# genlm/genlm-backend

Hardware: AMD Instinct MI355X
Metric: particles/sec + logprob-kernel HBM GB/s (% of 8 TB/s), 1024 particles gpt2 (higher is better)
Workload: dtype f32

## Files before the change

genlm-backend_amd/csrc/glb_kv.hip:

```cpp
#include <hip/hip_runtime.h>

#include <climits>

#include "../../include/glb.h"
#include "glb_common.hpp"

namespace {

__device__ inline uint64_t ctx_hash_step(uint64_t h, uint32_t v) {
  h ^= v;
  h *= 0x100000001b3ull;
  return h ^ (h >> 29);
}

__global__ __launch_bounds__(64) void match_rows_kernel(const int32_t *tok, const int64_t *st, const int32_t *len,
                                                        const int32_t *rep, const int32_t *n_groups, const int32_t *row_tok,
                                                        const int32_t *row_len, const uint64_t *row_hash, int32_t R,
                                                        int32_t cap, int32_t *out_old, uint64_t *out_hash) {
  const int u = blockIdx.x, lane = threadIdx.x;
  if (u >= *n_groups) return;
  const int i = rep[u];
  const int32_t L = len[i];
  const int32_t *t = tok + st[i];
  uint64_t h = 0xcbf29ce484222325ull, h_par = h;
// ... 499 lines not shown
  const int p0_new = a.pos[r], nn = a.n_new[r];
  const int64_t sr = a.row_of ? (int64_t)a.row_of[r] : (int64_t)r;
  char *out = a.out + ((((int64_t)r * a.T + t) * a.H + h) * DH + i * EPV) * ES;
  const bool bad = p0_new < 0 || nn < 1 || nn > a.T || (int64_t)p0_new + nn > a.cap || sr < 0 || sr >= a.n_slab_rows;
  if (bad || t >= nn) {
    if (j == 0) {
      float z[EPV];
#pragma unroll
      for (int k = 0; k < EPV; ++k) z[k] = bad ? __builtin_nanf("") : 0.0f;
      *reinterpret_cast<u32x4 *>(out) = pack16v<DT>(z);
    }
    return;
  }
  const int p_new = p0_new + t;
  float qf[EPV];
  unpack16<DT>(*reinterpret_cast<const u32x4 *>(a.q + ((int64_t)r * a.q_sr + (int64_t)h * a.q_sh + (int64_t)t * a.q_sp + i * EPV) * ES), qf);
  const char *kb = a.k_new + ((int64_t)r * a.k_sr + (int64_t)hk * a.k_sh + i * EPV) * ES;
  const char *vb = a.v_new + ((int64_t)r * a.v_sr + (int64_t)hk * a.v_sh + i * EPV) * ES;
  const int64_t slab_row = (sr * a.Hkv + hk) * a.cap;
  if (h == hk * G && j == 0) {
    *reinterpret_cast<u32x4 *>(a.k_slab + ((slab_row + p_new) * DH + i * EPV) * ES) = *reinterpret_cast<const u32x4 *>(kb + (int64_t)t * a.k_sp * ES);
    *reinterpret_cast<u32x4 *>(a.v_slab + ((slab_row + p_new) * DH + i * EPV) * ES) = *reinterpret_cast<const u32x4 *>(vb + (int64_t)t * a.v_sp * ES);
  }
  float m = -__builtin_huge_valf(), l = 0.0f, acc[EPV];
#pragma unroll
  for (int k = 0; k < EPV; ++k) acc[k] = 0.0f;
  for (int p0 = 0; p0 <= p_new; p0 += PP) {
    const int p = p0 + j;
    float kf[EPV], vf[EPV];
    if (p < p0_new) {
      unpack16<DT>(*reinterpret_cast<const u32x4 *>(a.k_slab + ((slab_row + p) * DH + i * EPV) * ES), kf);
      unpack16<DT>(*reinterpret_cast<const u32x4 *>(a.v_slab + ((slab_row + p) * DH + i * EPV) * ES), vf);
    } else {
      const int tn = p <= p_new ? p - p0_new : t;
      unpack16<DT>(*reinterpret_cast<const u32x4 *>(kb + (int64_t)tn * a.k_sp * ES), kf);
      unpack16<DT>(*reinterpret_cast<const u32x4 *>(vb + (int64_t)tn * a.v_sp * ES), vf);
    }
    float s = 0.0f;
#pragma unroll
    for (int k = 0; k < EPV; ++k) s = __builtin_fmaf(qf[k], kf[k], s);
#pragma unroll
    for (int o = 1; o < LP; o <<= 1) s += __shfl_xor(s, o, 64);
    if (p <= p_new) {
      s *= a.scale;
      const float m2 = fmaxf(m, s), c = __expf(m - m2), w = __expf(s - m2);
      l = l * c + w;
#pragma unroll
      for (int k = 0; k < EPV; ++k) acc[k] = __builtin_fmaf(acc[k], c, w * vf[k]);
      m = m2;
    }
  }
#pragma unroll
  for (int o = LP; o < 64; o <<= 1) {
    const float mo = __shfl_xor(m, o, 64), lo = __shfl_xor(l, o, 64);
    const float m2 = fmaxf(m, mo);
    const float c = m == m2 ? 1.0f : __expf(m - m2), co = mo == m2 ? 1.0f : __expf(mo - m2);
    l = l * c + lo * co;
#pragma unroll
    for (int k = 0; k < EPV; ++k) acc[k] = acc[k] * c + __shfl_xor(acc[k], o, 64) * co;
    m = m2;
  }
  if (j == 0) {
    const float inv = 1.0f / l;
#pragma unroll
    for (int k = 0; k < EPV; ++k) acc[k] *= inv;
    *reinterpret_cast<u32x4 *>(out) = pack16v<DT>(acc);
  }
}

template <int DT>
hipError_t launch_attention_chunk(const ChunkAttnArgs &a, int head_dim, hipStream_t s) {
  const dim3 grid((unsigned)((int64_t)a.n * a.H * a.T)), block(64);
  if (head_dim == 64) hipLaunchKernelGGL((slab_attention_chunk_kernel<DT, 64>), grid, block, 0, s, a);
  else if (head_dim == 128) hipLaunchKernelGGL((slab_attention_chunk_kernel<DT, 128>), grid, block, 0, s, a);
  else if (head_dim == 32) hipLaunchKernelGGL((slab_attention_chunk_kernel<DT, 32>), grid, block, 0, s, a);
  else if (head_dim == 16) hipLaunchKernelGGL((slab_attention_chunk_kernel<DT, 16>), grid, block, 0, s, a);
  else return hipErrorInvalidValue;
  return hipGetLastError();
}

struct ShortArgs {
  const char *q, *k, *v;
  const uint8_t *mask;
  char *out;
  int64_t q_sr, q_sh, q_sp, k_sr, k_sh, k_sp, v_sr, v_sh, v_sp, m_sr, m_sq;
  int32_t U, H, Hkv, Lq, Lk;
  float scale;
};

template <int DT, int DH>
__global__ __launch_bounds__(64) void short_attention_kernel(const ShortArgs a) {
  constexpr int ES = DT == GLB_F32 ? 4 : 2, EPV = 16 / ES, LP = DH / EPV, PP = 64 / LP;
  static_assert(LP >= 1 && LP <= 64 && PP * LP == 64, "head_dim / vector width must divide the wave");
  const int lane = threadIdx.x, j = lane / LP, i = lane - j * LP;
  const int t = blockIdx.x % a.Lq, uh = blockIdx.x / a.Lq, h = uh % a.H, u = uh / a.H;
  const int hk = h / (a.H / a.Hkv);
  float qf[EPV];
  unpack16<DT>(*reinterpret_cast<const u32x4 *>(a.q + ((int64_t)u * a.q_sr + (int64_t)h * a.q_sh + (int64_t)t * a.q_sp + i * EPV) * ES), qf);
  const uint8_t *mrow = a.mask ? a.mask + (int64_t)u * a.m_sr + (int64_t)t * a.m_sq : nullptr;
  const int last = mrow ? a.Lk - 1 : (t + a.Lk - a.Lq < a.Lk - 1 ? t + a.Lk - a.Lq : a.Lk - 1);
  const char *kb = a.k + ((int64_t)u * a.k_sr + (int64_t)hk * a.k_sh + i * EPV) * ES;
  const char *vb = a.v + ((int64_t)u * a.v_sr + (int64_t)hk * a.v_sh + i * EPV) * ES;
  float m = -__builtin_huge_valf(), l = 0.0f, acc[EPV];
#pragma unroll
  for (int k = 0; k < EPV; ++k) acc[k] = 0.0f;
  for (int p0 = 0; p0 <= last; p0 += PP) {
    const int p = p0 + j;
    const bool in = p <= last;
    const bool see = in && (mrow ? mrow[p] != 0 : true);
    float kf[EPV], vf[EPV];
    const int pc = in ? p : last;
    unpack16<DT>(*reinterpret_cast<const u32x4 *>(kb + (int64_t)pc * a.k_sp * ES), kf);
    unpack16<DT>(*reinterpret_cast<const u32x4 *>(vb + (int64_t)pc * a.v_sp * ES), vf);
    float s = 0.0f;
#pragma unroll
    for (int k = 0; k < EPV; ++k) s = __builtin_fmaf(qf[k], kf[k], s);
#pragma unroll
    for (int o = 1; o < LP; o <<= 1) s += __shfl_xor(s, o, 64);
    if (see) {
      s *= a.scale;
      const float m2 = fmaxf(m, s), c = __expf(m - m2), w = __expf(s - m2);
      l = l * c + w;
#pragma unroll
      for (int k = 0; k < EPV; ++k) acc[k] = __builtin_fmaf(acc[k], c, w * vf[k]);
      m = m2;
    }
  }
#pragma unroll
  for (int o = LP; o < 64; o <<= 1) {
    const float mo = __shfl_xor(m, o, 64), lo = __shfl_xor(l, o, 64);
    const float m2 = fmaxf(m, mo);
    const float c = m == m2 ? 1.0f : __expf(m - m2), co = mo == m2 ? 1.0f : __expf(mo - m2);
    l = l * c + lo * co;
#pragma unroll
    for (int k = 0; k < EPV; ++k) acc[k] = acc[k] * c + __shfl_xor(acc[k], o, 64) * co;
    m = m2;
  }
  if (j == 0) {
    const float inv = l > 0.0f ? 1.0f / l : 0.0f;
#pragma unroll
    for (int k = 0; k < EPV; ++k) acc[k] *= inv;
    *reinterpret_cast<u32x4 *>(a.out + ((((int64_t)u * a.Lq + t) * a.H + h) * DH + i * EPV) * ES) = pack16v<DT>(acc);
  }
}

template <int LP>
__device__ __forceinline__ float slot_sum(float v) {
  if constexpr (LP >= 2) v += __uint_as_float((uint32_t)__builtin_amdgcn_update_dpp(0, (int)__float_as_uint(v), 0xB1, 0xf, 0xf, false));
  if constexpr (LP >= 4) v += __uint_as_float((uint32_t)__builtin_amdgcn_update_dpp(0, (int)__float_as_uint(v), 0x4E, 0xf, 0xf, false));
  if constexpr (LP >= 8) v += __uint_as_float((uint32_t)__builtin_amdgcn_update_dpp(0, (int)__float_as_uint(v), 0x141, 0xf, 0xf, false));
  if constexpr (LP >= 16) v += __uint_as_float((uint32_t)__builtin_amdgcn_update_dpp(0, (int)__float_as_uint(v), 0x140, 0xf, 0xf, false));
  if constexpr (LP >= 32) v += __shfl_xor(v, 16, 64);
  if constexpr (LP >= 64) v += __shfl_xor(v, 32, 64);
  return v;
}

template <int DT, int DH, int KMAX>
__global__ __launch_bounds__(64) void short_attention_rows_kernel(const ShortArgs a) {
  constexpr int ES = DT == GLB_F32 ? 4 : 2, EPV = 16 / ES, LP = DH / EPV, PP = 64 / LP;
  static_assert(LP >= 1 && LP <= 64 && PP * LP == 64, "head_dim / vector width must divide the wave");
  constexpr bool KREG = KMAX * EPV <= 128;
  extern __shared__ float kv_lds[];
  const int lane = threadIdx.x, j = lane / LP, i = lane - j * LP;
  const int G = a.H / a.Hkv;
  const int hk = blockIdx.x % a.Hkv, u = blockIdx.x / a.Hkv;
  float *Ks = kv_lds, *Vs = KREG ? kv_lds : kv_lds + a.Lk * DH;
  const char *kb = a.k + ((int64_t)u * a.k_sr + (int64_t)hk * a.k_sh) * ES;
  const char *vb = a.v + ((int64_t)u * a.v_sr + (int64_t)hk * a.v_sh) * ES;
  const int nq = G * a.Lq;
  auto q_addr = [&](int qi) {
    const int qc = qi < nq ? qi : nq - 1;
    const int g = qc / a.Lq, t = qc - g * a.Lq;
    return a.q + ((int64_t)u * a.q_sr + (int64_t)(hk * G + g) * a.q_sh + (int64_t)t * a.q_sp + i * EPV) * ES;
  };
  u32x4 q_raw = *reinterpret_cast<const u32x4 *>(q_addr(j));
  float kr[KREG ? KMAX : 1][EPV];
  if constexpr (KREG) {
    u32x4 raw[KMAX];
#pragma unroll
    for (int p = 0; p < KMAX; ++p)
      raw[p] = *reinterpret_cast<const u32x4 *>(kb + ((int64_t)(p < a.Lk ? p : 0) * a.k_sp + i * EPV) * ES);
#pragma unroll
    for (int p = 0; p < KMAX; ++p) unpack16<DT>(raw[p], kr[p]);
  }
  for (int x = lane; x < a.Lk * LP; x += 64) {
    const int p = x / LP, c = x - p * LP;
    float vf[EPV];
    unpack16<DT>(*reinterpret_cast<const u32x4 *>(vb + ((int64_t)p * a.v_sp + c * EPV) * ES), vf);
#pragma unroll
    for (int k = 0; k < EPV; ++k) Vs[p * DH + c * EPV + k] = vf[k];
    if constexpr (!KREG) {
      float kf[EPV];
      unpack16<DT>(*reinterpret_cast<const u32x4 *>(kb + ((int64_t)p * a.k_sp + c * EPV) * ES), kf);
#pragma unroll
      for (int k = 0; k < EPV; ++k) Ks[p * DH + c * EPV + k] = kf[k];
    }
  }
  const uint32_t all_keys = a.Lk >= 32 ? 0xffffffffu : ((1u << a.Lk) - 1u);
  uint32_t *vis_t = reinterpret_cast<uint32_t *>(kv_lds + (KREG ? 1 : 2) * a.Lk * DH);
  for (int t = lane; t < a.Lq; t += 64) {
    uint32_t vis = 0;
    if (a.mask) {
      const uint8_t *mrow = a.mask + (int64_t)u * a.m_sr + (int64_t)t * a.m_sq;
      uint8_t mb[KMAX];
#pragma unroll
      for (int p = 0; p < KMAX; ++p) mb[p] = p < a.Lk ? mrow[p] : (uint8_t)0;
#pragma unroll
      for (int p = 0; p < KMAX; ++p) vis |= (mb[p] != 0 ? 1u : 0u) << p;
    } else {
      const int last = t + a.Lk - a.Lq;
      vis = last >= 31 ? 0xffffffffu : ((2u << last) - 1u);
    }
    vis_t[t] = vis & all_keys;
  }
  __syncthreads();
  for (int q0 = 0; q0 < nq; q0 += PP) {
    const int qi = q0 + j;
    const bool live = qi < nq;
    const int qc = live ? qi : nq - 1;
    const int g = qc / a.Lq, t = qc - g * a.Lq, h = hk * G + g;
    float qf[EPV];
    unpack16<DT>(q_raw, qf);
    if (q0 + PP < nq) q_raw = *reinterpret_cast<const u32x4 *>(q_addr(qi + PP));
    const uint32_t vis = vis_t[t];
    float sc[KMAX];
    float m = -__builtin_huge_valf();
#pragma unroll
    for (int p = 0; p < KMAX; ++p) {
      sc[p] = -__builtin_huge_valf();
      if (p < a.Lk) {
        float s = 0.0f;
        if constexpr (KREG) {
#pragma unroll
          for (int k = 0; k < EPV; ++k) s = __builtin_fmaf(qf[k], kr[p][k], s);
        } else {
          const float *kp = Ks + p * DH + i * EPV;
#pragma unroll
          for (int k = 0; k < EPV; ++k) s = __builtin_fmaf(qf[k], kp[k], s);
        }
        s = slot_sum<LP>(s) * a.scale;
        sc[p] = ((vis >> p) & 1u) ? s : -__builtin_huge_valf();
        m = fmaxf(m, sc[p]);
      }
    }
    float l = 0.0f, acc[EPV];
#pragma unroll
    for (int k = 0; k < EPV; ++k) acc[k] = 0.0f;
#pragma unroll
    for (int p = 0; p < KMAX; ++p) {
      if (p < a.Lk) {
        const float w = ((vis >> p) & 1u) ? __expf(sc[p] - m) : 0.0f;
        const float *vp = Vs + p * DH + i * EPV;
        l += w;
#pragma unroll
        for (int k = 0; k < EPV; ++k) acc[k] = __builtin_fmaf(w, vp[k], acc[k]);
      }
    }
    if (live) {
      const float inv = l > 0.0f ? 1.0f / l : 0.0f;
#pragma unroll
      for (int k = 0; k < EPV; ++k) acc[k] *= inv;
      *reinterpret_cast<u32x4 *>(a.out + ((((int64_t)u * a.Lq + t) * a.H + h) * DH + i * EPV) * ES) = pack16v<DT>(acc);
    }
  }
}

template <int DT, int DH>
hipError_t launch_short_rows(const ShortArgs &a, hipStream_t s) {
  const dim3 grid((unsigned)((int64_t)a.U * a.Hkv)), block(64);
  const size_t lds = (size_t)2 * a.Lk * DH * sizeof(float) + (size_t)a.Lq * sizeof(uint32_t);
  if (a.Lk <= 16) hipLaunchKernelGGL((short_attention_rows_kernel<DT, DH, 16>), grid, block, lds, s, a);
  else hipLaunchKernelGGL((short_attention_rows_kernel<DT, DH, 32>), grid, block, lds, s, a);
  return hipGetLastError();
}

template <int DT>
hipError_t launch_short_attention(const ShortArgs &a, int head_dim, hipStream_t s) {
  if (a.Lk <= 32 && a.Lq <= 2048 && (int64_t)a.U * a.Hkv <= 0x7fffffffll) {
    if (head_dim == 64) return launch_short_rows<DT, 64>(a, s);
    if (head_dim == 128) return launch_short_rows<DT, 128>(a, s);
    if (head_dim == 32) return launch_short_rows<DT, 32>(a, s);
    if (head_dim == 16) return launch_short_rows<DT, 16>(a, s);
    return hipErrorInvalidValue;
  }
  const dim3 grid((unsigned)((int64_t)a.U * a.H * a.Lq)), block(64);
  if (head_dim == 64) hipLaunchKernelGGL((short_attention_kernel<DT, 64>), grid, block, 0, s, a);
  else if (head_dim == 128) hipLaunchKernelGGL((short_attention_kernel<DT, 128>), grid, block, 0, s, a);
  else if (head_dim == 32) hipLaunchKernelGGL((short_attention_kernel<DT, 32>), grid, block, 0, s, a);
  else if (head_dim == 16) hipLaunchKernelGGL((short_attention_kernel<DT, 16>), grid, block, 0, s, a);
  else return hipErrorInvalidValue;
  return hipGetLastError();
}

struct PackedArgs {
  const char *q, *k, *v;
  char *out;
  const int32_t *plan;
  uint32_t *err;
  int64_t q_sr, q_sh, k_sr, k_sh, v_sr, v_sh;
  int32_t S, M, H, Hkv, max_keys;
  float scale;
};

template <int DT, int DH, int KMAX>
__global__ __launch_bounds__(64) void short_attention_packed_kernel(const PackedArgs a) {
  constexpr int ES = DT == GLB_F32 ? 4 : 2, EPV = 16 / ES, LP = DH / EPV, PP = 64 / LP;
  static_assert(LP >= 1 && LP <= 64 && PP * LP == 64, "head_dim / vector width must divide the wave");
  constexpr bool KREG = KMAX * EPV <= 128;
  extern __shared__ float kv_lds[];
  const int lane = threadIdx.x, j = lane / LP, i = lane - j * LP;
  const int G = a.H / a.Hkv;
  const int hk = blockIdx.x % a.Hkv, s = blockIdx.x / a.Hkv;
  if (s >= a.S) return;
  const int32_t *seg = a.plan + (int64_t)s * 4;
  const int64_t pre_start = seg[0], pre_len = seg[1], tail_start = seg[2], tail_len = seg[3];
  const int64_t n_keys = pre_len + tail_len;
  if (pre_len < 0 || tail_len < 1 || n_keys > a.max_keys || n_keys > KMAX || pre_start < 0 || pre_start + pre_len > a.M ||
      tail_start < 0 || tail_start + tail_len > a.M) {
    if (lane == 0 && hk == 0) atomicAdd(a.err, 1u);
    return;
  }
  const int Lk = (int)n_keys, Lq = (int)tail_len, pre = (int)pre_len;
  auto key_row = [&](int p) -> int64_t { return p < pre ? pre_start + p : tail_start + (p - pre); };
  float *Ks = kv_lds, *Vs = KREG ? kv_lds : kv_lds + Lk * DH;
  const char *kb = a.k + (int64_t)hk * a.k_sh * ES;
  const char *vb = a.v + (int64_t)hk * a.v_sh * ES;
  const int nq = G * Lq;
  auto q_addr = [&](int qi) {
    const int qc = qi < nq ? qi : nq - 1;
    const int g = qc / Lq, t = qc - g * Lq;
    return a.q + ((tail_start + t) * a.q_sr + (int64_t)(hk * G + g) * a.q_sh + i * EPV) * ES;
  };
  u32x4 q_raw = *reinterpret_cast<const u32x4 *>(q_addr(j));
  float kr[KREG ? KMAX : 1][EPV];
  if constexpr (KREG) {
    u32x4 raw[KMAX];
#pragma unroll
    for (int p = 0; p < KMAX; ++p)
      raw[p] = *reinterpret_cast<const u32x4 *>(kb + (key_row(p < Lk ? p : 0) * a.k_sr + i * EPV) * ES);
#pragma unroll
    for (int p = 0; p < KMAX; ++p) unpack16<DT>(raw[p], kr[p]);
  }
  for (int x = lane; x < Lk * LP; x += 64) {
    const int p = x / LP, c = x - p * LP;
    const int64_t row = key_row(p);
    float vf[EPV];
    unpack16<DT>(*reinterpret_cast<const u32x4 *>(vb + (row * a.v_sr + c * EPV) * ES), vf);
#pragma unroll
    for (int k = 0; k < EPV; ++k) Vs[p * DH + c * EPV + k] = vf[k];
    if constexpr (!KREG) {
      float kf[EPV];
      unpack16<DT>(*reinterpret_cast<const u32x4 *>(kb + (row * a.k_sr + c * EPV) * ES), kf);
#pragma unroll
      for (int k = 0; k < EPV; ++k) Ks[p * DH + c * EPV + k] = kf[k];
    }
  }
  const uint32_t all_keys = Lk >= 32 ? 0xffffffffu : ((1u << Lk) - 1u);
  uint32_t *vis_t = reinterpret_cast<uint32_t *>(kv_lds + (KREG ? 1 : 2) * Lk * DH);
  for (int t = lane; t < Lq; t += 64) {
    const int last = t + pre;
    const uint32_t vis = last >= 31 ? 0xffffffffu : ((2u << last) - 1u);
    vis_t[t] = vis & all_keys;
  }
  __syncthreads();
  for (int q0 = 0; q0 < nq; q0 += PP) {
    const int qi = q0 + j;
    const bool live = qi < nq;
    const int qc = live ? qi : nq - 1;
    const int g = qc / Lq, t = qc - g * Lq, h = hk * G + g;
    float qf[EPV];
    unpack16<DT>(q_raw, qf);
    if (q0 + PP < nq) q_raw = *reinterpret_cast<const u32x4 *>(q_addr(qi + PP));
    const uint32_t vis = vis_t[t];
    float sc[KMAX];
    float m = -__builtin_huge_valf();
#pragma unroll
    for (int p = 0; p < KMAX; ++p) {
      sc[p] = -__builtin_huge_valf();
      if (p < Lk) {
        float sv = 0.0f;
        if constexpr (KREG) {
#pragma unroll
          for (int k = 0; k < EPV; ++k) sv = __builtin_fmaf(qf[k], kr[p][k], sv);
        } else {
          const float *kp = Ks + p * DH + i * EPV;
#pragma unroll
          for (int k = 0; k < EPV; ++k) sv = __builtin_fmaf(qf[k], kp[k], sv);
        }
        sv = slot_sum<LP>(sv) * a.scale;
        sc[p] = ((vis >> p) & 1u) ? sv : -__builtin_huge_valf();
        m = fmaxf(m, sc[p]);
      }
    }
    float l = 0.0f, acc[EPV];
#pragma unroll
    for (int k = 0; k < EPV; ++k) acc[k] = 0.0f;
#pragma unroll
    for (int p = 0; p < KMAX; ++p) {
      if (p < Lk) {
        const float w = ((vis >> p) & 1u) ? __expf(sc[p] - m) : 0.0f;
        const float *vp = Vs + p * DH + i * EPV;
        l += w;
#pragma unroll
        for (int k = 0; k < EPV; ++k) acc[k] = __builtin_fmaf(w, vp[k], acc[k]);
      }
    }
    if (live) {
      const float inv = l > 0.0f ? 1.0f / l : 0.0f;
#pragma unroll
      for (int k = 0; k < EPV; ++k) acc[k] *= inv;
      *reinterpret_cast<u32x4 *>(a.out + (((tail_start + t) * a.H + h) * DH + i * EPV) * ES) = pack16v<DT>(acc);
    }
  }
}

template <int DT, int DH>
hipError_t launch_short_packed_dh(const PackedArgs &a, hipStream_t s) {
  const dim3 grid((unsigned)((int64_t)a.S * a.Hkv)), block(64);
  const size_t lds = (size_t)2 * a.max_keys * DH * sizeof(float) + (size_t)a.max_keys * sizeof(uint32_t);
  if (a.max_keys <= 16) hipLaunchKernelGGL((short_attention_packed_kernel<DT, DH, 16>), grid, block, lds, s, a);
  else hipLaunchKernelGGL((short_attention_packed_kernel<DT, DH, 32>), grid, block, lds, s, a);
  return hipGetLastError();
}

template <int DT>
hipError_t launch_short_packed(const PackedArgs &a, int head_dim, hipStream_t s) {
  if (head_dim == 64) return launch_short_packed_dh<DT, 64>(a, s);
  if (head_dim == 128) return launch_short_packed_dh<DT, 128>(a, s);
  if (head_dim == 32) return launch_short_packed_dh<DT, 32>(a, s);
  if (head_dim == 16) return launch_short_packed_dh<DT, 16>(a, s);
  return hipErrorInvalidValue;
}


template <typename VT>
__global__ void kv_append_kernel(VT *slab, const VT *rows, const int32_t *pos, const int32_t *row_of, int64_t n_rows,
                                 int64_t heads, int64_t cap, int64_t row_vecs, int64_t rows_stride_row,
                                 int64_t rows_stride_head) {
  const int64_t gid = (int64_t)blockIdx.x * blockDim.x + threadIdx.x;
  if (gid >= n_rows * heads * row_vecs) return;
  const int64_t x = gid % row_vecs, h = (gid / row_vecs) % heads, i = gid / (row_vecs * heads);
  const int64_t p = pos[i], r = row_of ? (int64_t)row_of[i] : i;
  if (p < 0 || p >= cap || r < 0) return;
  slab[((r * heads + h) * cap + p) * row_vecs + x] = rows[i * rows_stride_row + h * rows_stride_head + x];
}

template <typename VT>
__global__ void kv_gather_rows_kernel(const VT *const *src, VT *const *dst, int64_t n_rows, int64_t heads,
                                      int64_t row_vecs, int64_t src_cap, int64_t dst_cap, const int32_t *src_row_of,
                                      const int32_t *len_of) {
  const int t = blockIdx.y;
  const int64_t gid = (int64_t)blockIdx.x * blockDim.x + threadIdx.x;
  const int64_t per_row = heads * dst_cap * row_vecs;
  if (gid >= n_rows * per_row) return;
  const int64_t i = gid / per_row, r = gid % per_row;
  const int64_t x = r % row_vecs, p = (r / row_vecs) % dst_cap, h = r / (row_vecs * dst_cap);
  const int64_t sr = src_row_of[i];
  if (sr < 0 || p >= len_of[i] || p >= src_cap) return;
  dst[t][((i * heads + h) * dst_cap + p) * row_vecs + x] = src[t][((sr * heads + h) * src_cap + p) * row_vecs + x];
}

__global__ void gather_rows_i32_kernel(const int32_t *src, int64_t src_ld, const int32_t *row_of, int64_t n,
                                       int64_t width, int32_t *dst, int64_t dst_ld) {
  const int64_t gid = (int64_t)blockIdx.x * blockDim.x + threadIdx.x;
  if (gid >= n * width) return;
  const int64_t i = gid / width, j = gid % width;
  dst[i * dst_ld + j] = src[(int64_t)row_of[i] * src_ld + j];
}


}

extern "C" {

int glb_kv_append(void *slab, const void *new_rows, const int32_t *pos, const int32_t *row_of, int64_t n_rows,
                  int64_t heads, int64_t cap, int64_t head_dim, int64_t new_stride_row, int64_t new_stride_head,
                  int32_t elem_bytes, void *stream) {
  if (!slab || !new_rows || !pos) return glb::api_fail(GLB_EINVAL, "null pointer");
  if (n_rows <= 0 || heads <= 0 || cap <= 0 || head_dim <= 0) return glb::api_fail(GLB_EINVAL, "bad sizes");
  if (elem_bytes != 2 && elem_bytes != 4) return glb::api_fail(GLB_EINVAL, "elem_bytes must be 2 or 4");
  const int64_t rowb = head_dim * elem_bytes;
  hipStream_t s = (hipStream_t)stream;
  const bool wide = rowb % 16 == 0 && ((uintptr_t)slab) % 16 == 0 && ((uintptr_t)new_rows) % 16 == 0 &&
                    (new_stride_row * elem_bytes) % 16 == 0 && (new_stride_head * elem_bytes) % 16 == 0;
  if (wide) {
    const int64_t rv = rowb / 16, total = n_rows * heads * rv;
    hipLaunchKernelGGL(kv_append_kernel<uint4>, dim3(blocks_for(total, 256)), dim3(256), 0, s, (uint4 *)slab,
                       (const uint4 *)new_rows, pos, row_of, n_rows, heads, cap, rv, new_stride_row * elem_bytes / 16,
                       new_stride_head * elem_bytes / 16);
  } else if (elem_bytes == 4) {
    const int64_t total = n_rows * heads * head_dim;
    hipLaunchKernelGGL(kv_append_kernel<uint32_t>, dim3(blocks_for(total, 256)), dim3(256), 0, s, (uint32_t *)slab,
                       (const uint32_t *)new_rows, pos, row_of, n_rows, heads, cap, head_dim, new_stride_row, new_stride_head);
  } else {
    const int64_t total = n_rows * heads * head_dim;
    hipLaunchKernelGGL(kv_append_kernel<uint16_t>, dim3(blocks_for(total, 256)), dim3(256), 0, s, (uint16_t *)slab,
                       (const uint16_t *)new_rows, pos, row_of, n_rows, heads, cap, head_dim, new_stride_row, new_stride_head);
  }
  const hipError_t e = hipGetLastError();
  if (e != hipSuccess) return glb::api_hip_fail(e, "kv_append launch");
  return GLB_OK;
}

int glb_kv_gather_rows(const void *const *src, void *const *dst, int64_t n_tensors, int64_t n_rows, int64_t heads,
                       int64_t head_dim, int64_t src_cap, int64_t dst_cap, const int32_t *src_row_of,
                       const int32_t *len_of, int32_t elem_bytes, void *stream) {
  if (!src || !dst || !src_row_of || !len_of) return glb::api_fail(GLB_EINVAL, "null pointer");
  if (n_tensors <= 0 || n_tensors > 65535 || n_rows <= 0 || heads <= 0 || head_dim <= 0 || src_cap <= 0 || dst_cap <= 0)
    return glb::api_fail(GLB_EINVAL, "bad sizes");
  if (elem_bytes != 2 && elem_bytes != 4) return glb::api_fail(GLB_EINVAL, "elem_bytes must be 2 or 4");
  const int64_t rowb = head_dim * elem_bytes;
  hipStream_t s = (hipStream_t)stream;
  if (rowb % 16 == 0) {
    const int64_t rv = rowb / 16, total = n_rows * heads * dst_cap * rv;
    hipLaunchKernelGGL(kv_gather_rows_kernel<uint4>, dim3(blocks_for(total, 256), (unsigned)n_tensors), dim3(256), 0, s,
                       (const uint4 *const *)src, (uint4 *const *)dst, n_rows, heads, rv, src_cap, dst_cap,
                       src_row_of, len_of);
  } else if (elem_bytes == 4) {
    const int64_t total = n_rows * heads * dst_cap * head_dim;
    hipLaunchKernelGGL(kv_gather_rows_kernel<uint32_t>, dim3(blocks_for(total, 256), (unsigned)n_tensors), dim3(256), 0,
                       s, (const uint32_t *const *)src, (uint32_t *const *)dst, n_rows, heads, head_dim, src_cap,
                       dst_cap, src_row_of, len_of);
  } else {
    const int64_t total = n_rows * heads * dst_cap * head_dim;
    hipLaunchKernelGGL(kv_gather_rows_kernel<uint16_t>, dim3(blocks_for(total, 256), (unsigned)n_tensors), dim3(256), 0,
                       s, (const uint16_t *const *)src, (uint16_t *const *)dst, n_rows, heads, head_dim, src_cap,
                       dst_cap, src_row_of, len_of);
  }
  const hipError_t e = hipGetLastError();
  if (e != hipSuccess) return glb::api_hip_fail(e, "kv_gather_rows launch");
  return GLB_OK;
}

int glb_gather_rows_i32(const int32_t *src, int64_t src_ld, const int32_t *row_of, int64_t n, int64_t width,
                        int32_t *dst, int64_t dst_ld, void *stream) {
  if (!src || !row_of || !dst) return glb::api_fail(GLB_EINVAL, "null pointer");
  if (n <= 0 || width <= 0 || src_ld < width || dst_ld < width) return glb::api_fail(GLB_EINVAL, "bad sizes");
  hipLaunchKernelGGL(gather_rows_i32_kernel, dim3(blocks_for(n * width, 256)), dim3(256), 0, (hipStream_t)stream, src,
                     src_ld, row_of, n, width, dst, dst_ld);
  const hipError_t e = hipGetLastError();
  if (e != hipSuccess) return glb::api_hip_fail(e, "gather_rows_i32 launch");
  return GLB_OK;
}


int glb_slab_attention(const void *q, int64_t q_stride_row, int64_t q_stride_head, const void *k_new, int64_t k_stride_row,
                       int64_t k_stride_head, const void *v_new, int64_t v_stride_row, int64_t v_stride_head, void *k_slab,
                       void *v_slab, const int32_t *pos,
                       int64_t n_rows, int64_t heads, int64_t kv_heads, int64_t cap, int64_t head_dim, float scale,
                       int32_t dtype, void *out, void *stream) {
  if (!q || !k_new || !v_new || !k_slab || !v_slab || !pos || !out) return glb::api_fail(GLB_EINVAL, "glb_slab_attention: null pointer");
  if (dtype < GLB_F32 || dtype > GLB_F16) return glb::api_fail(GLB_EINVAL, "bad dtype %d", dtype);
  if (n_rows <= 0 || heads <= 0 || kv_heads <= 0 || cap <= 0 || heads % kv_heads || n_rows * heads > 0x7fffffffll)
    return glb::api_fail(GLB_EINVAL, "glb_slab_attention: bad sizes");
  if (head_dim != 16 && head_dim != 32 && head_dim != 64 && head_dim != 128)
    return glb::api_fail(GLB_EUNSUPPORTED, "glb_slab_attention: head_dim %lld (16, 32, 64 and 128 are built)", (long long)head_dim);
  const int es = dtype == GLB_F32 ? 4 : 2;
  if (((uintptr_t)q | (uintptr_t)k_new | (uintptr_t)v_new | (uintptr_t)k_slab | (uintptr_t)v_slab | (uintptr_t)out) % 16 ||
      (q_stride_row * es) % 16 || (q_stride_head * es) % 16 || (k_stride_row * es) % 16 || (k_stride_head * es) % 16 ||
      (v_stride_row * es) % 16 || (v_stride_head * es) % 16)
    return glb::api_fail(GLB_EINVAL, "glb_slab_attention: pointers and strides must be 16-byte aligned");
  AttnArgs a{};
  a.q = (const char *)q;
  a.k_new = (const char *)k_new;
  a.v_new = (const char *)v_new;
  a.k_slab = (char *)k_slab;
  a.v_slab = (char *)v_slab;
  a.out = (char *)out;
  a.pos = pos;
  a.q_sr = q_stride_row;
  a.q_sh = q_stride_head;
  a.k_sr = k_stride_row;
  a.k_sh = k_stride_head;
  a.v_sr = v_stride_row;
  a.v_sh = v_stride_head;
  a.R = (int32_t)n_rows;
  a.H = (int32_t)heads;
  a.Hkv = (int32_t)kv_heads;
  a.cap = (int32_t)cap;
  a.scale = scale;
  hipError_t e;
  switch (dtype) {
    case GLB_F32: e = launch_attention<GLB_F32>(a, (int)head_dim, (hipStream_t)stream); break;
    case GLB_BF16: e = launch_attention<GLB_BF16>(a, (int)head_dim, (hipStream_t)stream); break;
    default: e = launch_attention<GLB_F16>(a, (int)head_dim, (hipStream_t)stream); break;
  }
  if (e != hipSuccess) return glb::api_hip_fail(e, "slab_attention launch");
  return GLB_OK;
}

int glb_slab_attention_chunk(const void *q, const int64_t q_strides[3], const void *k_new, const int64_t k_strides[3],
                             const void *v_new, const int64_t v_strides[3], void *k_slab, void *v_slab, const int32_t *pos,
                             const int32_t *n_new, const int32_t *row_of, int64_t n_rows, int64_t n_slab_rows, int64_t heads,
                             int64_t kv_heads, int64_t cap, int64_t head_dim, int64_t max_new, float scale, int32_t dtype,
                             void *out, void *stream) {
  if (!q || !k_new || !v_new || !k_slab || !v_slab || !pos || !n_new || !out || !q_strides || !k_strides || !v_strides)
    return glb::api_fail(GLB_EINVAL, "glb_slab_attention_chunk: null pointer");
  if (dtype < GLB_F32 || dtype > GLB_F16) return glb::api_fail(GLB_EINVAL, "bad dtype %d", dtype);
  if (max_new < 1 || max_new > GLB_KV_CHUNK_MAX)
    return glb::api_fail(GLB_EINVAL, "glb_slab_attention_chunk: %lld query positions per row (1 .. %d)", (long long)max_new, GLB_KV_CHUNK_MAX);
  if (n_rows <= 0 || n_slab_rows <= 0 || heads <= 0 || kv_heads <= 0 || cap <= 0 || heads % kv_heads || cap > 0x7fffffffll ||
      n_slab_rows > 0x7fffffffll || n_rows * heads * max_new > 0x7fffffffll)
    return glb::api_fail(GLB_EINVAL, "glb_slab_attention_chunk: bad sizes");
  if (head_dim != 16 && head_dim != 32 && head_dim != 64 && head_dim != 128)
    return glb::api_fail(GLB_EUNSUPPORTED, "glb_slab_attention_chunk: head_dim %lld (16, 32, 64 and 128 are built)", (long long)head_dim);
  const int es = dtype == GLB_F32 ? 4 : 2;
  bool aligned = (((uintptr_t)q | (uintptr_t)k_new | (uintptr_t)v_new | (uintptr_t)k_slab | (uintptr_t)v_slab | (uintptr_t)out) % 16) == 0;
  for (int d = 0; d < 3; ++d) aligned = aligned && (q_strides[d] * es) % 16 == 0 && (k_strides[d] * es) % 16 == 0 && (v_strides[d] * es) % 16 == 0;
  if (!aligned) return glb::api_fail(GLB_EINVAL, "glb_slab_attention_chunk: pointers and strides must be 16-byte aligned");
  ChunkAttnArgs a{};
  a.q = (const char *)q;
  a.k_new = (const char *)k_new;
  a.v_new = (const char *)v_new;
  a.k_slab = (char *)k_slab;
  a.v_slab = (char *)v_slab;
  a.out = (char *)out;
  a.pos = pos;
  a.n_new = n_new;
  a.row_of = row_of;
  a.q_sr = q_strides[0], a.q_sh = q_strides[1], a.q_sp = q_strides[2];
  a.k_sr = k_strides[0], a.k_sh = k_strides[1], a.k_sp = k_strides[2];
  a.v_sr = v_strides[0], a.v_sh = v_strides[1], a.v_sp = v_strides[2];
  a.n = (int32_t)n_rows;
  a.H = (int32_t)heads;
  a.Hkv = (int32_t)kv_heads;
  a.cap = (int32_t)cap;
  a.T = (int32_t)max_new;
  a.n_slab_rows = (int32_t)n_slab_rows;
  a.scale = scale;
  hipError_t e;
  switch (dtype) {
    case GLB_F32: e = launch_attention_chunk<GLB_F32>(a, (int)head_dim, (hipStream_t)stream); break;
    case GLB_BF16: e = launch_attention_chunk<GLB_BF16>(a, (int)head_dim, (hipStream_t)stream); break;
    default: e = launch_attention_chunk<GLB_F16>(a, (int)head_dim, (hipStream_t)stream); break;
  }
  if (e != hipSuccess) return glb::api_hip_fail(e, "slab_attention_chunk launch");
  return GLB_OK;
}

int glb_match_rows(const int32_t *tokens, const int64_t *starts, const int32_t *lengths, const int32_t *rep,
                   const int32_t *n_groups, int64_t n, const int32_t *row_tok, const int32_t *row_len,
                   const uint64_t *row_hash, int64_t n_rows, int64_t cap, int32_t *out_old, uint64_t *out_hash,
                   void *stream) {
  if (!tokens || !starts || !lengths || !rep || !n_groups || !row_tok || !row_len || !row_hash || !out_old)
    return glb::api_fail(GLB_EINVAL, "glb_match_rows: null pointer");
  if (n <= 0 || n_rows <= 0 || cap <= 0 || n > 0x7fffffffll || n_rows > 0x7fffffffll || cap > 0x7fffffffll)
    return glb::api_fail(GLB_EINVAL, "glb_match_rows: bad sizes");
  hipLaunchKernelGGL(match_rows_kernel, dim3((unsigned)n), dim3(64), 0, (hipStream_t)stream, tokens, starts, lengths, rep,
                     n_groups, row_tok, row_len, row_hash, (int32_t)n_rows, (int32_t)cap, out_old, out_hash);
  const hipError_t e = hipGetLastError();
  if (e != hipSuccess) return glb::api_hip_fail(e, "match_rows launch");
  return GLB_OK;
}

int glb_match_prefix_rows(const int32_t *tokens, const int64_t *starts, const int32_t *lengths, const int32_t *rep,
                          const int32_t *n_groups, int64_t n, const int32_t *row_tok, const int32_t *row_len,
                          const uint64_t *row_hash, int64_t n_rows, int64_t cap, int32_t max_new, int32_t *out_old,
                          int32_t *out_keep, uint64_t *out_hash, void *stream) {
  (void)row_hash;
  if (!tokens || !starts || !lengths || !rep || !n_groups || !row_tok || !row_len || !out_old || !out_keep)
    return glb::api_fail(GLB_EINVAL, "glb_match_prefix_rows: null pointer");
  if (n <= 0 || n_rows <= 0 || cap <= 0 || n > 0x7fffffffll || n_rows > 0x3fffffffll || cap > 0x3fffffffll)
    return glb::api_fail(GLB_EINVAL, "glb_match_prefix_rows: bad sizes");
  if (max_new < 1 || max_new > GLB_KV_CHUNK_MAX)
    return glb::api_fail(GLB_EINVAL, "glb_match_prefix_rows: max_new %d outside 1 .. %d", max_new, GLB_KV_CHUNK_MAX);
  hipLaunchKernelGGL(match_prefix_rows_kernel, dim3((unsigned)n), dim3(64), 0, (hipStream_t)stream, tokens, starts, lengths,
                     rep, n_groups, row_tok, row_len, (int32_t)n_rows, (int32_t)cap, max_new, out_old, out_keep, out_hash);
  const hipError_t e = hipGetLastError();
  if (e != hipSuccess) return glb::api_hip_fail(e, "match_prefix_rows launch");
  return GLB_OK;
}

size_t glb_kv_plan_workspace(int64_t n, int64_t n_rows) {
  if (n <= 0 || n_rows <= 0) return 0;
  return (size_t)(2 * n_rows + n) * sizeof(int32_t) + 256;
}

static int kv_plan_launch(const glb_kv_plan_args *a, const int32_t *old_keep, int32_t *n_new_a, int32_t *n_new_row,
                          void *stream);

int glb_kv_plan(const glb_kv_plan_args *a, void *stream) { return kv_plan_launch(a, nullptr, nullptr, nullptr, stream); }

int glb_kv_plan_chunk(const glb_kv_plan_chunk_args *c, void *stream) {
  if (!c) return glb::api_fail(GLB_EINVAL, "glb_kv_plan_chunk: null args");
  if (c->struct_size != sizeof(glb_kv_plan_chunk_args))
    return glb::api_fail(GLB_EINVAL, "glb_kv_plan_chunk_args.struct_size %u != %zu (ABI mismatch)", c->struct_size,
                         sizeof(glb_kv_plan_chunk_args));
  if (!c->old_keep || !c->out_n_new_a || !c->out_n_new_of_row)
    return glb::api_fail(GLB_EINVAL, "glb_kv_plan_chunk: null old_keep / out_n_new_a / out_n_new_of_row");
  if (!c->plan.row_tok) return glb::api_fail(GLB_EINVAL, "glb_kv_plan_chunk: the row table is required (row lengths decide who keeps a row in place)");
  return kv_plan_launch(&c->plan, c->old_keep, c->out_n_new_a, c->out_n_new_of_row, stream);
}

static int kv_plan_launch(const glb_kv_plan_args *a, const int32_t *old_keep, int32_t *n_new_a, int32_t *n_new_row,
                          void *stream) {
  if (!a) return glb::api_fail(GLB_EINVAL, "glb_kv_plan: null args");
  if (a->struct_size != sizeof(glb_kv_plan_args))
    return glb::api_fail(GLB_EINVAL, "glb_kv_plan_args.struct_size %u != %zu (ABI mismatch)", a->struct_size, sizeof(glb_kv_plan_args));
  if (a->n <= 0 || a->n_rows <= 0 || a->cap <= 0 || a->n > 0x7fffffffll || a->n_rows > 0x7fffffffll || a->cap > 0x7fffffffll)
    return glb::api_fail(GLB_EINVAL, "glb_kv_plan: bad sizes");
  if (!a->group_of || !a->rep || !a->n_groups || !a->old_row || !a->lengths)
    return glb::api_fail(GLB_EINVAL, "glb_kv_plan: null input");
  if (!a->out_group_row || !a->out_logits_row || !a->out_rows_a || !a->out_ctx_a || !a->out_pos_a || !a->out_ctx_b ||
      !a->out_rows_b || !a->out_copy_src || !a->out_copy_len || !a->out_ctx_of_row || !a->out_pos_of_row || !a->out_head)
    return glb::api_fail(GLB_EINVAL, "glb_kv_plan: null output");
  if (a->row_tok && (!a->row_len || !a->row_hash || !a->group_hash || !a->tokens || !a->starts))
    return glb::api_fail(GLB_EINVAL, "glb_kv_plan: row table given without its columns / the contexts");
  if (!a->workspace || ((uintptr_t)a->workspace) % 4 || a->workspace_bytes < glb_kv_plan_workspace(a->n, a->n_rows))
    return glb::api_fail(GLB_ENOSPC, "glb_kv_plan: workspace %zu < %zu bytes", a->workspace_bytes, glb_kv_plan_workspace(a->n, a->n_rows));
  PlanArgs p{};
  p.n = (int32_t)a->n;
  p.R = (int32_t)a->n_rows;
  p.cap = (int32_t)a->cap;
  p.group_of = a->group_of;
  p.rep = a->rep;
  p.n_groups = a->n_groups;
  p.old_src = a->old_row;
  p.old_sel = a->old_row_by_context ? a->rep : nullptr;
  p.lengths = a->lengths;
  p.stamps = a->row_stamps;
  p.call_no = a->call_no;
  p.grp_row = a->out_group_row;
  p.inv = a->out_logits_row;
  p.rows_a = a->out_rows_a;
  p.reps_a = a->out_ctx_a;
// ... 118 lines not shown
```

Before: 142,700.

## Remap packed short attention so each lane slot owns a KV head

The packed short-attention kernel now assigns one KV head to each lane group (PP heads per wave) instead of one KV head per block. Each lane group loops over all of its queries itself. K stays in registers, V goes into per-lane LDS cells, with a few V rows kept in registers for f32 with KMAX=16. The shared visibility table and the __syncthreads are replaced by a per-query causal count. A KMAX=24 instantiation is also added. The aim is fewer blocks, no LDS staging barrier and better lane utilisation when queries per head are few, at the cost of serial query loops and higher register pressure.

```diff
diff --git a/genlm-backend_amd/csrc/glb_kv.hip b/genlm-backend_amd/csrc/glb_kv.hip
--- a/genlm-backend_amd/csrc/glb_kv.hip
+++ b/genlm-backend_amd/csrc/glb_kv.hip
@@ -825,93 +825,93 @@
   float scale;
 };
 
+template <int DT, int KMAX>
+constexpr int packed_v_regs() {
+  return DT == GLB_F32 && KMAX == 16 ? 4 : 0;
+}
+
 template <int DT, int DH, int KMAX>
 __global__ __launch_bounds__(64) void short_attention_packed_kernel(const PackedArgs a) {
   constexpr int ES = DT == GLB_F32 ? 4 : 2, EPV = 16 / ES, LP = DH / EPV, PP = 64 / LP;
   static_assert(LP >= 1 && LP <= 64 && PP * LP == 64, "head_dim / vector width must divide the wave");
-  constexpr bool KREG = KMAX * EPV <= 128;
-  extern __shared__ float kv_lds[];
+  constexpr bool KFLT = KMAX * EPV <= 128;
+  constexpr int VR = packed_v_regs<DT, KMAX>();
+  extern __shared__ u32x4 v_cells[];
   const int lane = threadIdx.x, j = lane / LP, i = lane - j * LP;
   const int G = a.H / a.Hkv;
-  const int hk = blockIdx.x % a.Hkv, s = blockIdx.x / a.Hkv;
+  const int n_w = (a.Hkv + PP - 1) / PP;
+  const int w = blockIdx.x % n_w, s = blockIdx.x / n_w;
   if (s >= a.S) return;
   const int32_t *seg = a.plan + (int64_t)s * 4;
   const int64_t pre_start = seg[0], pre_len = seg[1], tail_start = seg[2], tail_len = seg[3];
   const int64_t n_keys = pre_len + tail_len;
   if (pre_len < 0 || tail_len < 1 || n_keys > a.max_keys || n_keys > KMAX || pre_start < 0 || pre_start + pre_len > a.M ||
       tail_start < 0 || tail_start + tail_len > a.M) {
-    if (lane == 0 && hk == 0) atomicAdd(a.err, 1u);
+    if (lane == 0 && w == 0) atomicAdd(a.err, 1u);
     return;
   }
+  const int hk = w * PP + j;
+  if (hk >= a.Hkv) return;
   const int Lk = (int)n_keys, Lq = (int)tail_len, pre = (int)pre_len;
   auto key_row = [&](int p) -> int64_t { return p < pre ? pre_start + p : tail_start + (p - pre); };
-  float *Ks = kv_lds, *Vs = KREG ? kv_lds : kv_lds + Lk * DH;
-  const char *kb = a.k + (int64_t)hk * a.k_sh * ES;
-  const char *vb = a.v + (int64_t)hk * a.v_sh * ES;
+  const char *kb = a.k + ((int64_t)hk * a.k_sh + i * EPV) * ES;
+  const char *vb = a.v + ((int64_t)hk * a.v_sh + i * EPV) * ES;
+  const char *qb = a.q + ((int64_t)hk * G * a.q_sh + i * EPV) * ES;
   const int nq = G * Lq;
   auto q_addr = [&](int qi) {
-    const int qc = qi < nq ? qi : nq - 1;
-    const int g = qc / Lq, t = qc - g * Lq;
-    return a.q + ((tail_start + t) * a.q_sr + (int64_t)(hk * G + g) * a.q_sh + i * EPV) * ES;
+    const int g = qi / Lq, t = qi - g * Lq;
+    return qb + ((tail_start + t) * a.q_sr + (int64_t)g * a.q_sh) * ES;
   };
-  u32x4 q_raw = *reinterpret_cast<const u32x4 *>(q_addr(j));
-  float kr[KREG ? KMAX : 1][EPV];
-  if constexpr (KREG) {
-    u32x4 raw[KMAX];
-#pragma unroll
-    for (int p = 0; p < KMAX; ++p)
-      raw[p] = *reinterpret_cast<const u32x4 *>(kb + (key_row(p < Lk ? p : 0) * a.k_sr + i * EPV) * ES);
-#pragma unroll
-    for (int p = 0; p < KMAX; ++p) unpack16<DT>(raw[p], kr[p]);
-  }
-  for (int x = lane; x < Lk * LP; x += 64) {
-    const int p = x / LP, c = x - p * LP;
-    const int64_t row = key_row(p);
-    float vf[EPV];
-    unpack16<DT>(*reinterpret_cast<const u32x4 *>(vb + (row * a.v_sr + c * EPV) * ES), vf);
-#pragma unroll
-    for (int k = 0; k < EPV; ++k) Vs[p * DH + c * EPV + k] = vf[k];
-    if constexpr (!KREG) {
-      float kf[EPV];
-      unpack16<DT>(*reinterpret_cast<const u32x4 *>(kb + (row * a.k_sr + c * EPV) * ES), kf);
-#pragma unroll
-      for (int k = 0; k < EPV; ++k) Ks[p * DH + c * EPV + k] = kf[k];
-    }
-  }
-  const uint32_t all_keys = Lk >= 32 ? 0xffffffffu : ((1u << Lk) - 1u);
-  uint32_t *vis_t = reinterpret_cast<uint32_t *>(kv_lds + (KREG ? 1 : 2) * Lk * DH);
-  for (int t = lane; t < Lq; t += 64) {
-    const int last = t + pre;
-    const uint32_t vis = last >= 31 ? 0xffffffffu : ((2u << last) - 1u);
-    vis_t[t] = vis & all_keys;
-  }
-  __syncthreads();
-  for (int q0 = 0; q0 < nq; q0 += PP) {
-    const int qi = q0 + j;
-    const bool live = qi < nq;
-    const int qc = live ? qi : nq - 1;
-    const int g = qc / Lq, t = qc - g * Lq, h = hk * G + g;
+  u32x4 q_raw = *reinterpret_cast<const u32x4 *>(q_addr(0));
+  u32x4 kraw[KMAX];
+#pragma unroll
+  for (int p = 0; p < KMAX; ++p) kraw[p] = *reinterpret_cast<const u32x4 *>(kb + key_row(p < Lk ? p : 0) * a.k_sr * ES);
+  u32x4 *vc = v_cells + lane;
+  u32x4 vreg[VR > 0 ? VR : 1];
+#pragma unroll
+  for (int p = 0; p < VR; ++p) vreg[p] = *reinterpret_cast<const u32x4 *>(vb + key_row(p < Lk ? p : 0) * a.v_sr * ES);
+#pragma unroll
+  for (int p0 = VR; p0 < KMAX; p0 += 8) {
+    if (p0 < Lk) {
+      u32x4 vraw[8];
+#pragma unroll
+      for (int p = 0; p < 8; ++p)
+        if (p0 + p < KMAX) vraw[p] = *reinterpret_cast<const u32x4 *>(vb + key_row(p0 + p < Lk ? p0 + p : 0) * a.v_sr * ES);
+#pragma unroll
+      for (int p = 0; p < 8; ++p)
+        if (p0 + p < KMAX && p0 + p < Lk) vc[(p0 + p - VR) * 64] = vraw[p];
+    }
+  }
+  float kr[KFLT ? KMAX : 1][EPV];
+  if constexpr (KFLT) {
+#pragma unroll
+    for (int p = 0; p < KMAX; ++p) unpack16<DT>(kraw[p], kr[p]);
+  }
+  for (int qi = 0; qi < nq; ++qi) {
+    const int g = qi / Lq, t = qi - g * Lq, h = hk * G + g;
     float qf[EPV];
     unpack16<DT>(q_raw, qf);
-    if (q0 + PP < nq) q_raw = *reinterpret_cast<const u32x4 *>(q_addr(qi + PP));
-    const uint32_t vis = vis_t[t];
+    if (qi + 1 < nq) q_raw = *reinterpret_cast<const u32x4 *>(q_addr(qi + 1));
+    const int n_vis = pre + t + 1;
     float sc[KMAX];
     float m = -__builtin_huge_valf();
 #pragma unroll
     for (int p = 0; p < KMAX; ++p) {
       sc[p] = -__builtin_huge_valf();
-      if (p < Lk) {
+      if (p < n_vis) {
         float sv = 0.0f;
-        if constexpr (KREG) {
+        if constexpr (KFLT) {
 #pragma unroll
           for (int k = 0; k < EPV; ++k) sv = __builtin_fmaf(qf[k], kr[p][k], sv);
         } else {
-          const float *kp = Ks + p * DH + i * EPV;
-#pragma unroll
-          for (int k = 0; k < EPV; ++k) sv = __builtin_fmaf(qf[k], kp[k], sv);
+          float kf[EPV];
+          asm volatile("" : "+v"(kraw[p]));
+          unpack16<DT>(kraw[p], kf);
+#pragma unroll
+          for (int k = 0; k < EPV; ++k) sv = __builtin_fmaf(qf[k], kf[k], sv);
         }
         sv = slot_sum<LP>(sv) * a.scale;
-        sc[p] = ((vis >> p) & 1u) ? sv : -__builtin_huge_valf();
+        sc[p] = sv;
         m = fmaxf(m, sc[p]);
       }
     }
@@ -921,29 +921,39 @@
 #pragma unroll
     for (int p = 0; p < KMAX; ++p) {
       if (p < Lk) {
-        const float w = ((vis >> p) & 1u) ? __expf(sc[p] - m) : 0.0f;
-        const float *vp = Vs + p * DH + i * EPV;
-        l += w;
-#pragma unroll
-        for (int k = 0; k < EPV; ++k) acc[k] = __builtin_fmaf(w, vp[k], acc[k]);
-      }
-    }
-    if (live) {
-      const float inv = l > 0.0f ? 1.0f / l : 0.0f;
-#pragma unroll
-      for (int k = 0; k < EPV; ++k) acc[k] *= inv;
-      *reinterpret_cast<u32x4 *>(a.out + (((tail_start + t) * a.H + h) * DH + i * EPV) * ES) = pack16v<DT>(acc);
-    }
-  }
+        float vf[EPV];
+        unpack16<DT>(p < VR ? vreg[p < VR ? p : 0] : vc[(p - VR) * 64], vf);
+        float wgt = 0.0f;
+        if (p < n_vis) {
+          wgt = __expf(sc[p] - m);
+          l += wgt;
+        }
+#pragma unroll
+        for (int k = 0; k < EPV; ++k) acc[k] = __builtin_fmaf(wgt, vf[k], acc[k]);
+      }
+    }
+    const float inv = l > 0.0f ? 1.0f / l : 0.0f;
+#pragma unroll
+    for (int k = 0; k < EPV; ++k) acc[k] *= inv;
+    *reinterpret_cast<u32x4 *>(a.out + (((tail_start + t) * a.H + h) * DH + i * EPV) * ES) = pack16v<DT>(acc);
+  }
+}
+
+template <int DT, int DH, int KMAX>
+hipError_t launch_short_packed_form(const PackedArgs &a, hipStream_t s) {
+  constexpr int ES = DT == GLB_F32 ? 4 : 2, PP = 64 / (DH / (16 / ES));
+  const dim3 grid((unsigned)((int64_t)a.S * ((a.Hkv + PP - 1) / PP))), block(64);
+  constexpr int VR = packed_v_regs<DT, KMAX>();
+  const size_t lds = (size_t)(a.max_keys > VR ? a.max_keys - VR : 0) * 64 * 16;
+  hipLaunchKernelGGL((short_attention_packed_kernel<DT, DH, KMAX>), grid, block, lds, s, a);
+  return hipGetLastError();
 }
 
 template <int DT, int DH>
 hipError_t launch_short_packed_dh(const PackedArgs &a, hipStream_t s) {
-  const dim3 grid((unsigned)((int64_t)a.S * a.Hkv)), block(64);
-  const size_t lds = (size_t)2 * a.max_keys * DH * sizeof(float) + (size_t)a.max_keys * sizeof(uint32_t);
-  if (a.max_keys <= 16) hipLaunchKernelGGL((short_attention_packed_kernel<DT, DH, 16>), grid, block, lds, s, a);
-  else hipLaunchKernelGGL((short_attention_packed_kernel<DT, DH, 32>), grid, block, lds, s, a);
-  return hipGetLastError();
+  if (a.max_keys <= 16) return launch_short_packed_form<DT, DH, 16>(a, s);
+  if (a.max_keys <= 24) return launch_short_packed_form<DT, DH, 24>(a, s);
+  return launch_short_packed_form<DT, DH, 32>(a, s);
 }
 
 template <int DT>
```

Result: no change. 145,100, median of 6 (+1.7%).
